# marksgraham/ddpm-ood

Hardware: AMD Instinct MI355X
Metric: reconstructions/sec (whole node), FashionMNIST 32x32 (higher is better)
Workload: dtype f32 (split-f16 MFMA products, fp32 accumulate)

## Files before the change

ddpm_ood_amd/csrc/conv_direct.hip:

```cpp
#include <stdlib.h>

#include "common.h"

namespace ddpm {

template <int COB>
__global__ __launch_bounds__(256) void conv_direct_kernel(const ddpm_conv_desc a) {
  const int HWo = a.Ho * a.Wo, HWi = a.Hi * a.Wi;
  const int Cin = a.C1 + a.C2;
  const int T = a.ksize * a.ksize;
  const int pad = a.ksize == 3 ? 1 : 0;
  const int s = a.mode == DDPM_CONV_STRIDE2 ? 2 : 1;
  const bool up = a.mode == DDPM_CONV_UPSAMPLE2;
  const int Hv = up ? a.Ho : a.Hi, Wv = up ? a.Wo : a.Wi;

  const int p = blockIdx.x * 256 + threadIdx.x;
  const int n = blockIdx.z;
  const int co0 = blockIdx.y * COB;
  if (p >= HWo) return;
  const int ho = p / a.Wo, wo = p - ho * a.Wo;

  float acc[COB];
#pragma unroll
  for (int j = 0; j < COB; ++j) acc[j] = 0.f;

  for (int ci = 0; ci < Cin; ++ci) {
    const float *plane = (ci < a.C1) ? a.in1 + ((size_t)n * a.C1 + ci) * HWi
                                     : a.in2 + ((size_t)n * a.C2 + (ci - a.C1)) * HWi;
    float sc = 1.f, sh = 0.f;
    if (a.gscale) {
      sc = a.gscale[(size_t)n * Cin + ci];
      sh = a.gshift[(size_t)n * Cin + ci];
    }
    for (int kh = 0; kh < a.ksize; ++kh) {
      for (int kw = 0; kw < a.ksize; ++kw) {
        const int hv = ho * s + kh - pad, wv = wo * s + kw - pad;
        float v = 0.f;
        if (hv >= 0 && hv < Hv && wv >= 0 && wv < Wv) {
          v = up ? plane[(hv >> 1) * a.Wi + (wv >> 1)] : plane[hv * a.Wi + wv];
          if (a.gscale) v = v * sc + sh;
          if (a.act == DDPM_ACT_SILU) v = silu_fast(v);
          if (a.act == DDPM_ACT_RELU) v = fmaxf(v, 0.f);
        }
        const int t = kh * a.ksize + kw;
#pragma unroll
        for (int j = 0; j < COB; ++j) {
          const int co = (co0 + j < a.Cout) ? co0 + j : a.Cout - 1;
          acc[j] = fmaf(v, a.w_raw[((size_t)co * Cin + ci) * T + t], acc[j]);
        }
      }
    }
  }
#pragma unroll
  for (int j = 0; j < COB; ++j) {
    const int co = co0 + j;
    if (co < a.Cout) {
      const size_t idx = ((size_t)n * a.Cout + co) * HWo + p;
      float v = acc[j];
      if (a.bias) v += a.bias[co];
      if (a.chan_add) v += a.chan_add[(size_t)n * a.chan_add_stride + co];
      if (a.residual) v += a.residual[idx];
      if (a.out_act == DDPM_ACT_RELU) v = fmaxf(v, 0.f);
      a.out[idx] = v;
    }
  }
}

constexpr int kSC_CH = 8;

template <int NPOS>
__global__ __launch_bounds__(256) void conv_smallco_kernel(const ddpm_conv_desc a, int TH, int RS, int PS) {
  extern __shared__ __attribute__((aligned(16))) float tile[];
  const int HW = a.Ho * a.Wo;
  const int Cin = a.C1 + a.C2;
  const int tid = threadIdx.x;
  const int n = blockIdx.y;
  const int h0 = blockIdx.x * TH;
  const bool live = tid < TH * a.Wo;
  const int th = live ? tid / a.Wo : 0, tw = live ? tid - th * a.Wo : 0;

  int soff[NPOS];
#pragma unroll
  for (int j = 0; j < NPOS; ++j) {
    const int r = tid + 256 * j;
    soff[j] = -1;
    if (r < PS) {
      const int ir = r / RS, ic = r - ir * RS;
      const int hv = h0 + ir - 1, wv = ic - 1;
      if (hv >= 0 && hv < a.Hi && wv >= 0 && wv < a.Wi) soff[j] = hv * a.Wi + wv;
    }
  }
  float acc[4] = {0.f, 0.f, 0.f, 0.f};
  const int pix = th * RS + tw;

  float pre[NPOS][kSC_CH], psc[kSC_CH], psh[kSC_CH];
  auto fetch = [&](int c0) {
#pragma unroll
    for (int c = 0; c < kSC_CH; ++c) {
      const int ci = c0 + c;
      const bool okc = ci < Cin;
      const float *plane = !okc ? a.in1
                           : (ci < a.C1) ? a.in1 + ((size_t)n * a.C1 + ci) * HW
                                         : a.in2 + ((size_t)n * a.C2 + (ci - a.C1)) * HW;
#pragma unroll
      for (int j = 0; j < NPOS; ++j) pre[j][c] = (okc && soff[j] >= 0) ? plane[soff[j]] : 0.f;
      psc[c] = (okc && a.gscale) ? a.gscale[(size_t)n * Cin + ci] : 1.f;
      psh[c] = (okc && a.gscale) ? a.gshift[(size_t)n * Cin + ci] : 0.f;
    }
  };
  fetch(0);
  for (int c0 = 0; c0 < Cin; c0 += kSC_CH) {
    __syncthreads();
#pragma unroll
    for (int j = 0; j < NPOS; ++j) {
      const int r = tid + 256 * j;
      if (r < PS) {
#pragma unroll
        for (int c = 0; c < kSC_CH; ++c) {
          float v = 0.f;
          if (soff[j] >= 0 && c0 + c < Cin) {
            v = pre[j][c];
            if (a.gscale) v = v * psc[c] + psh[c];
            if (a.act == DDPM_ACT_SILU) v = silu_fast(v);
            if (a.act == DDPM_ACT_RELU) v = fmaxf(v, 0.f);
          }
          tile[c * PS + r] = v;
        }
      }
    }
    __syncthreads();
    if (c0 + kSC_CH < Cin) fetch(c0 + kSC_CH);
#pragma unroll
    for (int c = 0; c < kSC_CH; ++c) {
      const int ci = c0 + c;
      if (ci < Cin) {
        float x[9];
#pragma unroll
        for (int kh = 0; kh < 3; ++kh)
#pragma unroll
          for (int kw = 0; kw < 3; ++kw) x[kh * 3 + kw] = tile[c * PS + pix + kh * RS + kw];
        for (int co = 0; co < a.Cout; ++co) {
          const float *w = a.w_raw + ((size_t)co * Cin + ci) * 9;
#pragma unroll
          for (int t = 0; t < 9; ++t) acc[co] = fmaf(x[t], w[t], acc[co]);
        }
      }
    }
  }
  const int p = (h0 + th) * a.Wo + tw;
  for (int co = 0; co < a.Cout && live; ++co) {
    const size_t idx = ((size_t)n * a.Cout + co) * HW + p;
    float v = acc[co];
    if (a.bias) v += a.bias[co];
    if (a.chan_add) v += a.chan_add[(size_t)n * a.chan_add_stride + co];
    if (a.residual) v += a.residual[idx];
    if (a.out_act == DDPM_ACT_RELU) v = fmaxf(v, 0.f);
    a.out[idx] = v;
  }
}

constexpr int kSW_NJ = 7;
constexpr int kSW_PPL = 4;

template <int NWV>
__global__ __launch_bounds__(64 * NWV) void conv_smallco_wave_kernel(const ddpm_conv_desc a, int TH, int RS, int PS) {
  extern __shared__ __attribute__((aligned(16))) float lds[];
  const int HW = a.Ho * a.Wo;
  const int Cin = a.C1 + a.C2;
  const int tid = threadIdx.x, lane = tid & 63, wave = __builtin_amdgcn_readfirstlane(tid >> 6);
  const int n = blockIdx.y;
  const int h0 = blockIdx.x * TH;
  float *plane_lds = lds + wave * 2 * PS;

  int soff[kSW_NJ];
#pragma unroll
  for (int j = 0; j < kSW_NJ; ++j) {
    const int r = lane + 64 * j;
    soff[j] = -1;
    if (r < PS) {
      const int ir = r / RS, ic = r - ir * RS;
      const int hv = h0 + ir - 1, wv = ic - 1;
      if (hv >= 0 && hv < a.Hi && wv >= 0 && wv < a.Wi) soff[j] = hv * a.Wi + wv;
    }
  }
  int pix[kSW_PPL];
#pragma unroll
  for (int k = 0; k < kSW_PPL; ++k) {
    const int q = lane + 64 * k;
    const int th = q / a.Wo, tw = q - th * a.Wo;
    pix[k] = (q < TH * a.Wo) ? th * RS + tw : 0;
  }
  float acc[kSW_PPL][4];
#pragma unroll
  for (int k = 0; k < kSW_PPL; ++k)
#pragma unroll
    for (int c = 0; c < 4; ++c) acc[k][c] = 0.f;

  float pre[2][kSW_NJ], psc[2] = {1.f, 1.f}, psh[2] = {0.f, 0.f};
  auto fetch = [&](int slot, int ci) {
    const float *plane = (ci < a.C1) ? a.in1 + ((size_t)n * a.C1 + ci) * HW
                                     : a.in2 + ((size_t)n * a.C2 + (ci - a.C1)) * HW;
#pragma unroll
    for (int j = 0; j < kSW_NJ; ++j) pre[slot][j] = soff[j] >= 0 ? plane[soff[j]] : 0.f;
    if (a.gscale) {
      psc[slot] = a.gscale[(size_t)n * Cin + ci];
      psh[slot] = a.gshift[(size_t)n * Cin + ci];
    }
  };
  auto consume = [&](int slot, int ci, int buf) {
    float *pl = plane_lds + buf * PS;
#pragma unroll
    for (int j = 0; j < kSW_NJ; ++j) {
      const int r = lane + 64 * j;
      if (r < PS) {
        float v = 0.f;
        if (soff[j] >= 0) {
          v = pre[slot][j];
          if (a.gscale) v = v * psc[slot] + psh[slot];
          if (a.act == DDPM_ACT_SILU) v = silu_fast(v);
          if (a.act == DDPM_ACT_RELU) v = fmaxf(v, 0.f);
        }
        pl[r] = v;
      }
    }
    if (ci + 2 * NWV < Cin) fetch(slot, ci + 2 * NWV);
    float wreg[4][9];
#pragma unroll
    for (int co = 0; co < 4; ++co) {
      const float *w = a.w_raw + ((size_t)min(co, a.Cout - 1) * Cin + ci) * 9;
#pragma unroll
      for (int t = 0; t < 9; ++t) wreg[co][t] = w[t];
    }
#pragma unroll
    for (int k = 0; k < kSW_PPL; ++k) {
      float x[9];
#pragma unroll
      for (int kh = 0; kh < 3; ++kh)
#pragma unroll
        for (int kw = 0; kw < 3; ++kw) x[kh * 3 + kw] = pl[pix[k] + kh * RS + kw];
#pragma unroll
      for (int co = 0; co < 4; ++co)
        if (co < a.Cout) {
#pragma unroll
          for (int t = 0; t < 9; ++t) acc[k][co] = fmaf(x[t], wreg[co][t], acc[k][co]);
        }
    }
  };
  if (wave < Cin) fetch(0, wave);
  if (wave + NWV < Cin) fetch(1, wave + NWV);
  for (int ci = wave; ci < Cin; ci += 2 * NWV) {
    consume(0, ci, 0);
    if (ci + NWV < Cin) consume(1, ci + NWV, 1);
  }
  float *red = lds + NWV * 2 * PS;
#pragma unroll
  for (int k = 0; k < kSW_PPL; ++k)
#pragma unroll
    for (int c = 0; c < 4; ++c) red[(wave * 256 + lane + 64 * k) * 4 + c] = acc[k][c];
  __syncthreads();
  if (tid < TH * a.Wo) {
    const int th = tid / a.Wo, tw = tid - th * a.Wo;
    const int p = (h0 + th) * a.Wo + tw;
    for (int co = 0; co < a.Cout; ++co) {
      float v = red[(0 * 256 + tid) * 4 + co];
#pragma unroll
      for (int wv = 1; wv < NWV; ++wv) v += red[(wv * 256 + tid) * 4 + co];
      const size_t idx = ((size_t)n * a.Cout + co) * HW + p;
      if (a.bias) v += a.bias[co];
      if (a.chan_add) v += a.chan_add[(size_t)n * a.chan_add_stride + co];
      if (a.residual) v += a.residual[idx];
      if (a.out_act == DDPM_ACT_RELU) v = fmaxf(v, 0.f);
      a.out[idx] = v;
    }
  }
}

template <int CIN>
__global__ __launch_bounds__(256) void conv_smallci_kernel(const ddpm_conv_desc a) {
  const int HW = a.Ho * a.Wo;
  const int p = blockIdx.x * 256 + threadIdx.x;
  const int n = blockIdx.y;
  if (p >= HW) return;
  const int ho = p / a.Wo, wo = p - ho * a.Wo;
  float x[CIN * 9];
#pragma unroll
  for (int ci = 0; ci < CIN; ++ci) {
    const float *plane = a.in1 + ((size_t)n * CIN + ci) * HW;
#pragma unroll
    for (int kh = 0; kh < 3; ++kh)
#pragma unroll
      for (int kw = 0; kw < 3; ++kw) {
        const int hv = ho + kh - 1, wv = wo + kw - 1;
        x[ci * 9 + kh * 3 + kw] = (hv >= 0 && hv < a.Hi && wv >= 0 && wv < a.Wi) ? plane[hv * a.Wi + wv] : 0.f;
      }
  }
  float *dst = a.out + (size_t)n * a.Cout * HW + p;
  const int cpz = (a.Cout + gridDim.z - 1) / gridDim.z, co_end = min(a.Cout, ((int)blockIdx.z + 1) * cpz);
  extern __shared__ float2 wred[];
  const bool emit = a.stats_out != nullptr;
  const int lane = threadIdx.x & 63, wave = threadIdx.x >> 6;
#pragma unroll 4
  for (int co = blockIdx.z * cpz; co < co_end; ++co) {
    const float *w = a.w_raw + (size_t)co * CIN * 9;
    float acc = 0.f;
#pragma unroll
    for (int k = 0; k < CIN * 9; ++k) acc = fmaf(x[k], w[k], acc);
    if (a.bias) acc += a.bias[co];
    dst[(size_t)co * HW] = acc;
    if (emit) {
      const float mean = wave_sum_dpp_last_lane(acc);
      const float mu = __builtin_bit_cast(float, __builtin_amdgcn_readlane(__builtin_bit_cast(int, mean), 63)) * (1.f / 64.f);
      const float dv = acc - mu;
      const float q = wave_sum_dpp_last_lane(dv * dv);
      if (lane == 63) wred[(co - blockIdx.z * cpz) * 4 + wave] = make_float2(mu, q);
    }
  }
  if (emit) {
    __syncthreads();
    const int parts = HW / 256;
    for (int c = threadIdx.x; c < co_end - (int)blockIdx.z * cpz; c += 256) {
      const float2 w0 = wred[c * 4], w1 = wred[c * 4 + 1], w2 = wred[c * 4 + 2], w3 = wred[c * 4 + 3];
      const float m01 = 0.5f * (w0.x + w1.x), d01 = w1.x - w0.x, q01 = (w0.y + w1.y) + d01 * d01 * 32.f;
      const float m23 = 0.5f * (w2.x + w3.x), d23 = w3.x - w2.x, q23 = (w2.y + w3.y) + d23 * d23 * 32.f;
      const float mm = 0.5f * (m01 + m23), dd = m23 - m01, qq = (q01 + q23) + dd * dd * 64.f;
      const int co = blockIdx.z * cpz + c;
      *reinterpret_cast<float2 *>(a.stats_out + (((size_t)n * a.Cout + co) * parts + blockIdx.x) * 2) = make_float2(mm, qq);
    }
  }
}

static bool smallci_supported(const ddpm_conv_desc &d) {
  const bool on = sw().convin_fast;
  return on && d.C2 == 0 && d.C1 >= 1 && d.C1 <= 4 && d.ksize == 3 && d.mode == DDPM_CONV_NORMAL && !d.gscale &&
         d.act == DDPM_ACT_NONE && !d.chan_add && !d.residual && d.out_act == DDPM_ACT_NONE && d.Cout >= 16 &&
         d.Di <= 1 && d.Do <= 1 && d.dims != 3;
}

static int smallci_stats_parts(const ddpm_conv_desc &d) {
  const int HW = d.Ho * d.Wo;
  if (!smallci_supported(d) || HW % 256 || HW / 256 > 8) return 0;
  return HW / 256;
}

static bool smallco_supported(const ddpm_conv_desc &d, int &TH, int &RS, int &PS) {
  if (d.Cout > 4 || d.ksize != 3 || d.mode != DDPM_CONV_NORMAL || d.Wo > 256 || d.Di > 1 || d.Do > 1) return false;
  TH = 0;
  for (int th = 256 / d.Wo; th >= 1; --th)
    if (d.Ho % th == 0) { TH = th; break; }
  if (TH == 0 || 2 * TH * d.Wo < 256) return false;
  RS = d.Wo + 2;
  PS = (TH + 2) * RS;
  return PS <= 512;
}

int launch_conv_direct(const ddpm_conv_desc &d, hipStream_t s) {
  DDPM_CHECK_ARG(d.w_raw != nullptr, "conv_direct: w_raw is NULL");
  DDPM_CHECK_ARG(d.ksize == 1 || d.ksize == 3, "conv_direct: ksize must be 1 or 3");
  DDPM_CHECK_ARG(d.B <= 65535, "conv_direct: batch > 65535");
  const int HWo = d.Ho * d.Wo;
  const double cin = d.C1 + d.C2, taps = d.ksize * d.ksize;
  const int Cin_i = d.C1 + d.C2;
  int TH, RS, PS;
  if (smallco_supported(d, TH, RS, PS)) {
    ProfScope prof(s, "conv3x3_small_cout", 2.0 * d.B * HWo * d.Cout * cin * 9,
                   4.0 * ((double)d.B * cin * HWo + (double)d.B * HWo * d.Cout + d.Cout * cin * 9));
    dim3 grid(d.Ho / TH, d.B);
    const bool wave_ok = sw().convout_wave;
    if (wave_ok && PS <= 64 * kSW_NJ && Cin_i >= 16) {
      const long w16_max = sw().convout_w16_maxwg;
      const long w16_wgs = w16_max >= 0 ? w16_max : 2L * device_cus();
      if ((long)grid.x * grid.y <= w16_wgs && Cin_i >= 64) {
        const size_t lds_w = ((size_t)16 * 2 * PS + 16 * 256 * 4) * sizeof(float);
        static bool attr_done = false;
        if (!attr_done) {
          (void)hipFuncSetAttribute(reinterpret_cast<const void *>(&conv_smallco_wave_kernel<16>), hipFuncAttributeMaxDynamicSharedMemorySize, 160 * 1024);
          attr_done = true;
        }
        hipLaunchKernelGGL(conv_smallco_wave_kernel<16>, grid, dim3(1024), lds_w, s, d, TH, RS, PS);
        DDPM_CHECK_LAUNCH();
        return 0;
      }
      const size_t lds_w = ((size_t)4 * 2 * PS + 4 * 256 * 4) * sizeof(float);
      hipLaunchKernelGGL(conv_smallco_wave_kernel<4>, grid, dim3(256), lds_w, s, d, TH, RS, PS);
      DDPM_CHECK_LAUNCH();
      return 0;
    }
    const size_t lds = (size_t)kSC_CH * PS * sizeof(float);
    if (PS <= 256)
      hipLaunchKernelGGL(conv_smallco_kernel<1>, grid, dim3(256), lds, s, d, TH, RS, PS);
    else
      hipLaunchKernelGGL(conv_smallco_kernel<2>, grid, dim3(256), lds, s, d, TH, RS, PS);
    DDPM_CHECK_LAUNCH();
    return 0;
  }
  if (smallci_supported(d)) {
    ProfScope prof(s, "conv3x3_small_cin", 2.0 * d.B * HWo * d.Cout * cin * 9,
                   4.0 * ((double)d.B * cin * HWo + (double)d.B * HWo * d.Cout + d.Cout * cin * 9));
    const long blocks = (long)((HWo + 255) / 256) * d.B;
    int zs = 1;
    const long zblk = sw().convin_blocks_per_cu;
    while (zs < 8 && blocks * zs * 2 <= device_cus() * zblk && d.Cout / (zs * 2) >= 16) zs *= 2;
    dim3 grid((HWo + 255) / 256, d.B, zs);
    ddpm_conv_desc dk = d;
    if (smallci_stats_parts(d) == 0) dk.stats_out = nullptr;
    const size_t lds = dk.stats_out ? (size_t)((d.Cout + zs - 1) / zs) * 4 * sizeof(float2) : 0;
    switch (d.C1) {
      case 1: hipLaunchKernelGGL(conv_smallci_kernel<1>, grid, dim3(256), lds, s, dk); break;
      case 2: hipLaunchKernelGGL(conv_smallci_kernel<2>, grid, dim3(256), lds, s, dk); break;
      case 3: hipLaunchKernelGGL(conv_smallci_kernel<3>, grid, dim3(256), lds, s, dk); break;
      default: hipLaunchKernelGGL(conv_smallci_kernel<4>, grid, dim3(256), lds, s, dk); break;
    }
    DDPM_CHECK_LAUNCH();
    return 0;
  }
  ProfScope prof(s, "conv_direct", 2.0 * d.B * HWo * d.Cout * cin * taps,
                 4.0 * ((double)d.B * cin * d.Hi * d.Wi + (double)d.B * HWo * d.Cout * (d.residual ? 2 : 1) +
                        d.Cout * cin * taps));
  if (d.Cout <= 4) {
    dim3 grid((HWo + 255) / 256, d.Cout, d.B);
    hipLaunchKernelGGL(conv_direct_kernel<1>, grid, dim3(256), 0, s, d);
  } else {
    dim3 grid((HWo + 255) / 256, (d.Cout + 7) / 8, d.B);
    hipLaunchKernelGGL(conv_direct_kernel<8>, grid, dim3(256), 0, s, d);
  }
  DDPM_CHECK_LAUNCH();
  return 0;
}

bool conv_direct_supported(const ddpm_conv_desc &) { return true; }

int conv_direct_stats_parts(const ddpm_conv_desc &d) {
  int TH, RS, PS;
  return d.mode == DDPM_CONV_NORMAL && !smallco_supported(d, TH, RS, PS) ? smallci_stats_parts(d) : 0;
}

}
```

Measured before the change: 1077.

## Add vectorized four-pixel-per-thread kernels for small-Cin and small-Cout 3x3 convs

Adds two new kernel variants that have each thread compute four adjacent output pixels using float4 loads and stores. The small-Cout wave kernel stages rows in LDS with vector loads and reuses a 3x6 input window across pixels. The small-Cin kernel runs one wave per block, reads weights from the constant address space, computes the norm statistics with row-level DPP reductions, and raises the block-per-CU budget used for the channel split. The aim is to cut redundant input loads and index arithmetic in the stem and output convolutions, at the cost of more registers per thread and extra alignment and shape conditions for dispatch.

```diff
diff --git a/ddpm_ood_amd/csrc/conv_direct.hip b/ddpm_ood_amd/csrc/conv_direct.hip
--- a/ddpm_ood_amd/csrc/conv_direct.hip
+++ b/ddpm_ood_amd/csrc/conv_direct.hip
@@ -1,4 +1,7 @@
+#include <stdint.h>
 #include <stdlib.h>
+
+#include <type_traits>
 
 #include "common.h"
 
@@ -275,6 +278,138 @@
   }
 }
 
+typedef float f32x4 __attribute__((ext_vector_type(4)));
+constexpr int kSV_NJ = 2;
+
+template <int COUT>
+__global__ __launch_bounds__(256) void conv_smallco_wave_vec_kernel(const ddpm_conv_desc a, int TH, int RS, int PS) {
+  constexpr int NWV = 4;
+  extern __shared__ __attribute__((aligned(16))) float lds[];
+  const int HW = a.Ho * a.Wo, W4 = a.Wo >> 2;
+  const int Cin = a.C1 + a.C2;
+  const int tid = threadIdx.x, lane = tid & 63, wave = __builtin_amdgcn_readfirstlane(tid >> 6);
+  const int n = blockIdx.y;
+  const int h0 = blockIdx.x * TH;
+  float *plane_lds = lds + wave * 2 * PS;
+
+  int goff[kSV_NJ], loff[kSV_NJ];
+#pragma unroll
+  for (int j = 0; j < kSV_NJ; ++j) {
+    const int f = lane + 64 * j;
+    goff[j] = loff[j] = -1;
+    if (f < (TH + 2) * W4) {
+      const int ir = f / W4, c4 = f - ir * W4;
+      const int hv = h0 + ir - 1;
+      loff[j] = ir * RS + 4 + 4 * c4;
+      if (hv >= 0 && hv < a.Hi) goff[j] = hv * a.Wi + 4 * c4;
+    }
+  }
+  for (int r = lane; r < 2 * (TH + 2); r += 64) {
+    float *row = plane_lds + (r / (TH + 2)) * PS + (r % (TH + 2)) * RS;
+    row[3] = 0.f;
+    row[a.Wo + 4] = 0.f;
+  }
+  const int q0 = 4 * lane;
+  const bool live = q0 < TH * a.Wo;
+  const int th = live ? q0 / a.Wo : 0, tw = live ? q0 - th * a.Wo : 0;
+  const int pix = th * RS + tw + 3;
+  float acc[4][COUT];
+#pragma unroll
+  for (int k = 0; k < 4; ++k)
+#pragma unroll
+    for (int c = 0; c < COUT; ++c) acc[k][c] = 0.f;
+
+  float4 pre[2][kSV_NJ];
+  float psc[2] = {1.f, 1.f}, psh[2] = {0.f, 0.f};
+  auto fetch = [&](int slot, int ci) {
+    const float *plane = (ci < a.C1) ? a.in1 + ((size_t)n * a.C1 + ci) * HW
+                                     : a.in2 + ((size_t)n * a.C2 + (ci - a.C1)) * HW;
+#pragma unroll
+    for (int j = 0; j < kSV_NJ; ++j)
+      pre[slot][j] = goff[j] >= 0 ? *reinterpret_cast<const float4 *>(plane + goff[j]) : make_float4(0.f, 0.f, 0.f, 0.f);
+    if (a.gscale) {
+      psc[slot] = a.gscale[(size_t)n * Cin + ci];
+      psh[slot] = a.gshift[(size_t)n * Cin + ci];
+    }
+  };
+  auto activate = [&](float v, int slot) {
+    if (a.gscale) v = v * psc[slot] + psh[slot];
+    if (a.act == DDPM_ACT_SILU) v = silu_fast(v);
+    if (a.act == DDPM_ACT_RELU) v = fmaxf(v, 0.f);
+    return v;
+  };
+  auto consume = [&](int slot, int ci, int buf) {
+    float *pl = plane_lds + buf * PS;
+#pragma unroll
+    for (int j = 0; j < kSV_NJ; ++j) {
+      if (loff[j] >= 0) {
+        float4 v = make_float4(0.f, 0.f, 0.f, 0.f);
+        if (goff[j] >= 0) {
+          v.x = activate(pre[slot][j].x, slot);
+          v.y = activate(pre[slot][j].y, slot);
+          v.z = activate(pre[slot][j].z, slot);
+          v.w = activate(pre[slot][j].w, slot);
+        }
+        *reinterpret_cast<float4 *>(pl + loff[j]) = v;
+      }
+    }
+    if (ci + 2 * NWV < Cin) fetch(slot, ci + 2 * NWV);
+    float wreg[COUT][9];
+#pragma unroll
+    for (int co = 0; co < COUT; ++co) {
+      const float *w = a.w_raw + ((size_t)co * Cin + ci) * 9;
+#pragma unroll
+      for (int t = 0; t < 9; ++t) wreg[co][t] = w[t];
+    }
+    float seg[3][6];
+#pragma unroll
+    for (int kh = 0; kh < 3; ++kh) {
+      const float *row = pl + pix + kh * RS;
+      const f32x4 mid = *reinterpret_cast<const f32x4 *>(row + 1);
+      seg[kh][0] = row[0];
+      seg[kh][1] = mid[0];
+      seg[kh][2] = mid[1];
+      seg[kh][3] = mid[2];
+      seg[kh][4] = mid[3];
+      seg[kh][5] = row[5];
+    }
+#pragma unroll
+    for (int k = 0; k < 4; ++k)
+#pragma unroll
+      for (int co = 0; co < COUT; ++co)
+#pragma unroll
+        for (int t = 0; t < 9; ++t) acc[k][co] = fmaf(seg[t / 3][k + t % 3], wreg[co][t], acc[k][co]);
+  };
+  if (wave < Cin) fetch(0, wave);
+  if (wave + NWV < Cin) fetch(1, wave + NWV);
+  for (int ci = wave; ci < Cin; ci += 2 * NWV) {
+    consume(0, ci, 0);
+    if (ci + NWV < Cin) consume(1, ci + NWV, 1);
+  }
+  __syncthreads();
+  float *red = lds;
+#pragma unroll
+  for (int k = 0; k < 4; ++k)
+#pragma unroll
+    for (int c = 0; c < COUT; ++c) red[(wave * 256 + q0 + k) * 4 + c] = acc[k][c];
+  __syncthreads();
+  if (tid < TH * a.Wo) {
+    const int oh = tid / a.Wo, ow = tid - oh * a.Wo;
+    const int p = (h0 + oh) * a.Wo + ow;
+    for (int co = 0; co < COUT; ++co) {
+      float v = red[(0 * 256 + tid) * 4 + co];
+#pragma unroll
+      for (int wv = 1; wv < NWV; ++wv) v += red[(wv * 256 + tid) * 4 + co];
+      const size_t idx = ((size_t)n * a.Cout + co) * HW + p;
+      if (a.bias) v += a.bias[co];
+      if (a.chan_add) v += a.chan_add[(size_t)n * a.chan_add_stride + co];
+      if (a.residual) v += a.residual[idx];
+      if (a.out_act == DDPM_ACT_RELU) v = fmaxf(v, 0.f);
+      a.out[idx] = v;
+    }
+  }
+}
+
 template <int CIN>
 __global__ __launch_bounds__(256) void conv_smallci_kernel(const ddpm_conv_desc a) {
   const int HW = a.Ho * a.Wo;
@@ -325,6 +460,99 @@
       const float mm = 0.5f * (m01 + m23), dd = m23 - m01, qq = (q01 + q23) + dd * dd * 64.f;
       const int co = blockIdx.z * cpz + c;
       *reinterpret_cast<float2 *>(a.stats_out + (((size_t)n * a.Cout + co) * parts + blockIdx.x) * 2) = make_float2(mm, qq);
+    }
+  }
+}
+
+template <int CTRL>
+__device__ __forceinline__ float dpp_add_partner(float v) {
+  return v + __builtin_bit_cast(float, __builtin_amdgcn_update_dpp(0, __builtin_bit_cast(int, v), CTRL, 0xf, 0xf, true));
+}
+__device__ __forceinline__ float row16_allsum(float v) {
+  v = dpp_add_partner<0xB1>(v);
+  v = dpp_add_partner<0x4E>(v);
+  v = dpp_add_partner<0x141>(v);
+  v = dpp_add_partner<0x140>(v);
+  return v;
+}
+
+template <int CIN, bool BIAS>
+__global__ __launch_bounds__(64) void conv_smallci_vec_kernel(const ddpm_conv_desc a) {
+  constexpr int G = CIN == 1 ? 8 : (CIN == 2 ? 4 : (CIN == 3 ? 2 : 1));
+  const int HW = a.Ho * a.Wo;
+  const int lane = threadIdx.x;
+  const int p = blockIdx.x * 256 + 4 * lane;
+  const int n = blockIdx.y;
+  const int ho = p / a.Wo, wo = p - ho * a.Wo;
+  float x[CIN][3][6];
+#pragma unroll
+  for (int ci = 0; ci < CIN; ++ci) {
+    const float *plane = a.in1 + ((size_t)n * CIN + ci) * HW;
+#pragma unroll
+    for (int kh = 0; kh < 3; ++kh)
+#pragma unroll
+      for (int c = 0; c < 6; ++c) {
+        const int hv = ho + kh - 1, wv = wo + c - 1;
+        x[ci][kh][c] = (hv >= 0 && hv < a.Hi && wv >= 0 && wv < a.Wi) ? plane[hv * a.Wi + wv] : 0.f;
+      }
+  }
+  float *dst = a.out + (size_t)n * a.Cout * HW + p;
+  const int cpz = (a.Cout + gridDim.z - 1) / gridDim.z, co_beg = blockIdx.z * cpz, co_end = min(a.Cout, co_beg + cpz);
+  typedef __attribute__((address_space(4))) float const_float;
+  const const_float *wts = (const const_float *)a.w_raw, *bias = (const const_float *)a.bias;
+  extern __shared__ float2 wred[];
+  const bool emit = a.stats_out != nullptr;
+  auto channels = [&](int co0, auto gc) {
+    constexpr int GG = decltype(gc)::value;
+    float acc[GG][4], wv[GG][CIN * 9], bv[GG];
+#pragma unroll
+    for (int g = 0; g < GG; ++g) {
+#pragma unroll
+      for (int i = 0; i < CIN * 9; ++i) wv[g][i] = wts[(size_t)(co0 + g) * CIN * 9 + i];
+      bv[g] = BIAS ? bias[co0 + g] : 0.f;
+    }
+#pragma unroll
+    for (int g = 0; g < GG; ++g) {
+      const float *w = wv[g];
+#pragma unroll
+      for (int k = 0; k < 4; ++k) {
+        float v = 0.f;
+#pragma unroll
+        for (int ci = 0; ci < CIN; ++ci)
+#pragma unroll
+          for (int kh = 0; kh < 3; ++kh)
+#pragma unroll
+            for (int kw = 0; kw < 3; ++kw) v = fmaf(x[ci][kh][k + kw], w[ci * 9 + kh * 3 + kw], v);
+        acc[g][k] = v;
+      }
+      if (BIAS) {
+#pragma unroll
+        for (int k = 0; k < 4; ++k) acc[g][k] += bv[g];
+      }
+      *reinterpret_cast<float4 *>(dst + (size_t)(co0 + g) * HW) = make_float4(acc[g][0], acc[g][1], acc[g][2], acc[g][3]);
+    }
+    if (emit) {
+#pragma unroll
+      for (int g = 0; g < GG; ++g) {
+        const float mu = row16_allsum((acc[g][1] + acc[g][0]) + (acc[g][3] + acc[g][2])) * (1.f / 64.f);
+        const float d0 = acc[g][0] - mu, d1 = acc[g][1] - mu, d2 = acc[g][2] - mu, d3 = acc[g][3] - mu;
+        const float q = row16_allsum((d1 * d1 + d0 * d0) + (d3 * d3 + d2 * d2));
+        if ((lane & 15) == 15) wred[(co0 + g - co_beg) * 4 + (lane >> 4)] = make_float2(mu, q);
+      }
+    }
+  };
+  int co = co_beg;
+  for (; co + G <= co_end; co += G) channels(co, std::integral_constant<int, G>{});
+  for (; co < co_end; ++co) channels(co, std::integral_constant<int, 1>{});
+  if (emit) {
+    __syncthreads();
+    const int parts = HW / 256;
+    for (int c = lane; c < co_end - co_beg; c += 64) {
+      const float2 w0 = wred[c * 4], w1 = wred[c * 4 + 1], w2 = wred[c * 4 + 2], w3 = wred[c * 4 + 3];
+      const float m01 = 0.5f * (w0.x + w1.x), d01 = w1.x - w0.x, q01 = (w0.y + w1.y) + d01 * d01 * 32.f;
+      const float m23 = 0.5f * (w2.x + w3.x), d23 = w3.x - w2.x, q23 = (w2.y + w3.y) + d23 * d23 * 32.f;
+      const float mm = 0.5f * (m01 + m23), dd = m23 - m01, qq = (q01 + q23) + dd * dd * 64.f;
+      *reinterpret_cast<float2 *>(a.stats_out + (((size_t)n * a.Cout + co_beg + c) * parts + blockIdx.x) * 2) = make_float2(mm, qq);
     }
   }
 }
@@ -380,6 +608,19 @@
         DDPM_CHECK_LAUNCH();
         return 0;
       }
+      const bool aligned16 = reinterpret_cast<uintptr_t>(d.in1) % 16 == 0 && (d.C2 == 0 || reinterpret_cast<uintptr_t>(d.in2) % 16 == 0);
+      if (d.Wo % 4 == 0 && aligned16 && (TH + 2) * (d.Wo / 4) <= 64 * kSV_NJ) {
+        const int RSv = d.Wo + 8, PSv = (TH + 2) * RSv;
+        const size_t lds_v = (size_t)max(4 * 2 * PSv, 4 * 256 * 4) * sizeof(float);
+        switch (d.Cout) {
+          case 1: hipLaunchKernelGGL(conv_smallco_wave_vec_kernel<1>, grid, dim3(256), lds_v, s, d, TH, RSv, PSv); break;
+          case 2: hipLaunchKernelGGL(conv_smallco_wave_vec_kernel<2>, grid, dim3(256), lds_v, s, d, TH, RSv, PSv); break;
+          case 3: hipLaunchKernelGGL(conv_smallco_wave_vec_kernel<3>, grid, dim3(256), lds_v, s, d, TH, RSv, PSv); break;
+          default: hipLaunchKernelGGL(conv_smallco_wave_vec_kernel<4>, grid, dim3(256), lds_v, s, d, TH, RSv, PSv); break;
+        }
+        DDPM_CHECK_LAUNCH();
+        return 0;
+      }
       const size_t lds_w = ((size_t)4 * 2 * PS + 4 * 256 * 4) * sizeof(float);
       hipLaunchKernelGGL(conv_smallco_wave_kernel<4>, grid, dim3(256), lds_w, s, d, TH, RS, PS);
       DDPM_CHECK_LAUNCH();
@@ -397,13 +638,28 @@
     ProfScope prof(s, "conv3x3_small_cin", 2.0 * d.B * HWo * d.Cout * cin * 9,
                    4.0 * ((double)d.B * cin * HWo + (double)d.B * HWo * d.Cout + d.Cout * cin * 9));
     const long blocks = (long)((HWo + 255) / 256) * d.B;
+    const bool vec = d.Wo % 4 == 0 && HWo % 256 == 0 && reinterpret_cast<uintptr_t>(d.out) % 16 == 0;
     int zs = 1;
-    const long zblk = sw().convin_blocks_per_cu;
+    const long zblk = sw().convin_blocks_per_cu * (vec ? 4 : 1);
     while (zs < 8 && blocks * zs * 2 <= device_cus() * zblk && d.Cout / (zs * 2) >= 16) zs *= 2;
     dim3 grid((HWo + 255) / 256, d.B, zs);
     ddpm_conv_desc dk = d;
     if (smallci_stats_parts(d) == 0) dk.stats_out = nullptr;
     const size_t lds = dk.stats_out ? (size_t)((d.Cout + zs - 1) / zs) * 4 * sizeof(float2) : 0;
+    if (vec) {
+#define DDPM_SMALLCI_VEC(CI)                                                                          \
+  if (d.bias) hipLaunchKernelGGL((conv_smallci_vec_kernel<CI, true>), grid, dim3(64), lds, s, dk); \
+  else hipLaunchKernelGGL((conv_smallci_vec_kernel<CI, false>), grid, dim3(64), lds, s, dk)
+      switch (d.C1) {
+        case 1: DDPM_SMALLCI_VEC(1); break;
+        case 2: DDPM_SMALLCI_VEC(2); break;
+        case 3: DDPM_SMALLCI_VEC(3); break;
+        default: DDPM_SMALLCI_VEC(4); break;
+      }
+#undef DDPM_SMALLCI_VEC
+      DDPM_CHECK_LAUNCH();
+      return 0;
+    }
     switch (d.C1) {
       case 1: hipLaunchKernelGGL(conv_smallci_kernel<1>, grid, dim3(256), lds, s, dk); break;
       case 2: hipLaunchKernelGGL(conv_smallci_kernel<2>, grid, dim3(256), lds, s, dk); break;
```

New measurement: 1086, median of 6. About the same (+0.8%).
